# raulmur/ORB_SLAM

Hardware: AMD Instinct MI355X
Metric: frames/s ORB extract+match @640x480, 1000 kp (higher is better)
Workload: dtype u8; 1 GPU; vga: 640x480 grayscale stream, 8 levels, nFeatures 1000, S-blocks frames, extract + Hamming top-2 match vs previous frame (BASELINE.json configs[1] + the frame-to-frame match of the metric); resident_frames_per_gpu=2048, lanes=4, parity_checked_frames=0, parity_mismatches=0, library_build_id=e7130e2d92184036, lane_placement=2

## Files before the change

### orb_slam_amd/csrc/k_select.hip

```cpp
#include <algorithm>
#include <type_traits>

#include "orbx_device.h"
#include "orbx_launch.h"

namespace orbx {

struct QuotaLds { int *nkeys, *nret; uint8_t *thr, *done; };

__global__ __launch_bounds__(64) void k_quota(Batch b) {
    extern __shared__ __attribute__((aligned(16))) uint8_t smem[];
    const DevGeom& g = b.g;
    QuotaLds q;
    q.nkeys = reinterpret_cast<int*>(smem);
    q.nret = q.nkeys + g.quota_cells;
    q.thr = reinterpret_cast<uint8_t*>(q.nret + g.quota_cells);
    q.done = q.thr + g.quota_cells;
    const int frame = blockIdx.x / g.nlevels, level = blockIdx.x - frame * g.nlevels;
    const int lane = (int)threadIdx.x;
    const LevelGeom& L = g.lv[level];
    const CellGeom* cg = b.cells + L.cell_base;
    const CellState* cs = b.cstate + (long long)frame * g.nbands_total;
    CellSel* sel = b.csel + (long long)frame * g.ncells_total + L.cell_base;
    const int nCells = L.ncells, nfc = L.nfeat_cell;
    int dist = 0, nomore = 0;
    for (int c = lane; c < nCells; c += 64) {
        const CellGeom cgc = cg[c];
        int n_hi = 0, n_lo = 0;
        for (int k = 0; k < cgc.nbands; k++) { const CellState t = cs[cgc.band0 + k]; n_hi += t.n_hi; n_lo += t.n_lo; }
        const bool fallback = n_hi <= 3;
        const int nk = cgc.skipped ? 0 : (fallback ? n_lo : n_hi);
        q.thr[c] = (uint8_t)(cgc.skipped || !fallback ? g.fast_th : 7);
        q.nkeys[c] = nk;
        if (cgc.skipped) { q.nret[c] = 0; q.done[c] = 0; }
        else if (nk > nfc) { q.nret[c] = nfc; q.done[c] = 0; }
        else { q.nret[c] = nk; dist += nfc - nk; q.done[c] = 1; nomore++; }
    }
    int nToDistribute = wave_sum(dist), nNoMore = wave_sum(nomore);
    while (nToDistribute > 0 && nNoMore < nCells) {
        const int nNew = nfc + (int)ceilf((float)nToDistribute / (float)(nCells - nNoMore));
        dist = 0; nomore = 0;
        for (int c = lane; c < nCells; c += 64) {
            if (q.done[c]) continue;
            const int nk = q.nkeys[c];
            if (nk > nNew) q.nret[c] = nNew;
            else { q.nret[c] = nk; dist += nNew - nk; q.done[c] = 1; nomore++; }
        }
        nToDistribute = wave_sum(dist);
        nNoMore += wave_sum(nomore);
    }
    int total = 0;
    for (int c0 = 0; c0 < nCells; c0 += 64) total += (c0 + lane < nCells) ? q.nret[c0 + lane] : 0;
    total = wave_sum(total);
    const bool bad = total > L.sel_cap;
    int base = 0;
    for (int c0 = 0; c0 < nCells; c0 += 64) {
        const int c = c0 + lane;
        const int v = c < nCells ? q.nret[c] : 0;
        const int incl = wave_scan_inclusive(v);
        if (c < nCells) {
            CellSel r;
            r.thr = q.thr[c]; r.nkeys = q.nkeys[c];
            r.nretain = bad ? 0 : v;
            r.out_off = bad ? 0 : base + incl - v;
            sel[c] = r;
        }
        base += __builtin_amdgcn_readlane(incl, 63);
    }
    if (lane == 0) {
        if (bad) b.status[frame] = ORBX_ERR_CAPACITY;
        b.level_total[frame * MAX_LEVELS + level] = bad ? 0 : total;
    }
}

struct RespGreater {
    __host__ __device__ constexpr bool operator()(const Cand& x, const Cand& y) const { return x.resp > y.resp; }
};


__device__ __forceinline__ int mask_rank(unsigned long long m) {
// ... 152 lines not shown
            const int Iy = (p[step] - p[-step]) * 2 + (p[step - 1] - p[-step - 1]) + (p[step + 1] - p[-step + 1]);
            a += Ix * Ix;
            bb += Iy * Iy;
            c += Ix * Iy;
        }
    if (fp_contract) {
        const float cc = (float)c * (float)c, sum = (float)a + (float)bb;
        return __builtin_fmaf(-sum, 0.04f * sum, __builtin_fmaf((float)a, (float)bb, -cc)) * scale_sq_sq;
    }
    return ((float)a * (float)bb - (float)c * (float)c - 0.04f * ((float)a + (float)bb) * ((float)a + (float)bb)) * scale_sq_sq;
}

constexpr int SEL_SMALL = 384;
__host__ __device__ constexpr int sel_wave_bytes(int entries) { return (entries * ((int)sizeof(Cand) + 4) + 16 + 15) & ~15; }
template <bool GATHER>
__device__ __forceinline__ bool cell_select_body(const Batch& b, int frame, int cell, int level, uint8_t* smem, int lds_entries, int min_entries, int lane) {
    const DevGeom& g = b.g;
    const LevelGeom& L = g.lv[level];
    const CellGeom cgeo = b.cells[cell];
    const CellSel s = b.csel[(long long)frame * g.ncells_total + cell];
    if (s.nretain <= 0) return true;
    const CellState* bst = b.cstate + (long long)frame * g.nbands_total + cgeo.band0;
    const BandGeom* bgs = b.bands + cgeo.band0;
    Cand* lbase = b.cand + (long long)frame * g.frame_cands + L.cand_base;
    Cand* c = lbase + cgeo.cand_off;
    int n_all = 0;
    for (int k = 0; k < cgeo.nbands; k++) n_all += bst[k].n_all;
    if (n_all < min_entries || (n_all > lds_entries && lds_entries < g.sel_lds_entries)) return false;
    Cand* out = b.sel + (long long)frame * g.frame_sel + L.sel_base + s.out_off;
    const float thr = (float)s.thr;
    long long stride;
    const uint8_t* img = plain_plane<GATHER>(b, L, level, frame, stride);
    if (n_all > lds_entries) {
        if (lane == 0) {
            int m = 0;
            for (int k = 0; k < cgeo.nbands; k++) {
                const Cand* bc = lbase + bgs[k].cand_off;
                const int nb = bst[k].n_all;
                for (int i = 0; i < nb; i++) { const Cand e = bc[i]; if (e.resp >= thr) c[m++] = e; }
            }
            if (g.score_type == ORBX_HARRIS_SCORE)
                for (int i = 0; i < m; i++) c[i].resp = harris_response(img, stride, c[i].pos & 0xFFFF, c[i].pos >> 16, g.fp_contract);
            if (m > s.nretain) std::nth_element(c, c + s.nretain, c + m, RespGreater());
            const int keep = min(m, s.nretain);
            for (int i = 0; i < keep; i++) out[i] = c[i];
        }
        return true;
    }
    Cand* lst = reinterpret_cast<Cand*>(smem);
    uint16_t* lpos = reinterpret_cast<uint16_t*>(smem + (size_t)lds_entries * sizeof(Cand));
    uint16_t* rpos = lpos + lds_entries;
    const unsigned long long lt = (1ull << lane) - 1ull;
    int m = 0;
    for (int k = 0; k < cgeo.nbands; k++) {
        const Cand* bc = lbase + bgs[k].cand_off;
        const int nb = bst[k].n_all;
        for (int base = 0; base < nb; base += 256) {
            Cand e4[4];
#pragma unroll
            for (int k = 0; k < 4; k++) {
                const int i = base + 64 * k + lane;
                e4[k].pos = 0; e4[k].resp = -1.f;
                if (i < nb) e4[k] = bc[i];
            }
#pragma unroll
            for (int k = 0; k < 4; k++) {
                if (base + 64 * k >= nb) break;
                const int i = base + 64 * k + lane;
                const bool pass = i < nb && e4[k].resp >= thr;
                const unsigned long long mk = __ballot(pass);
                if (pass) lst[m + __popcll(mk & lt)] = e4[k];
                m += __popcll(mk);
            }
        }
    }
    wave_lds_fence();
    if (g.score_type == ORBX_HARRIS_SCORE) {
        for (int i = lane; i < m; i += 64) lst[i].resp = harris_response(img, stride, lst[i].pos & 0xFFFF, lst[i].pos >> 16, g.fp_contract);
        wave_lds_fence();
    }
    if (m > s.nretain) wave_nth_element(lst, 0, s.nretain, m, lpos, rpos, lane);
    const int keep = min(m, s.nretain);
    for (int i = lane; i < keep; i += 64) out[i] = lst[i];
    return true;
}

template <bool GATHER>
__device__ __forceinline__ void k_cell_select_body(const Batch& b, int lds_entries) {
    extern __shared__ __attribute__((aligned(16))) uint8_t smem[];
    const DevGeom& g = b.g;
    const int wave = wave_id(), lane = (int)threadIdx.x & 63;
    const int id = (int)blockIdx.x * 4 + wave;
    if (id >= b.nframes * g.ncells_total) return;
    const int frame = id / g.ncells_total, cell = id - frame * g.ncells_total;
    const bool done = cell_select_body<GATHER>(b, frame, cell, find_level(g.cell_bases, cell), smem + wave * sel_wave_bytes(lds_entries), lds_entries, 0, lane);
    if (lane == 0) b.long_cells[id] = done ? 0 : 1;
}
__global__ __launch_bounds__(256) void k_cell_select(Batch b, int lds_entries) { k_cell_select_body<false>(b, lds_entries); }
__global__ __launch_bounds__(256) void k_cell_select_gather(Batch b, int lds_entries) { k_cell_select_body<true>(b, lds_entries); }
#ifndef ORBX_SEL_LONG_CHUNK
#define ORBX_SEL_LONG_CHUNK 8
#endif
constexpr int SEL_LONG_CHUNK = ORBX_SEL_LONG_CHUNK, SEL_LONG_WAVES = 4;
__host__ __device__ constexpr int sel_long_bytes(int entries) {
    int m = 0;
    for (int share = 1; share <= 4; share++) { const int v = share * sel_wave_bytes((entries + share - 1) / share); m = v > m ? v : m; }
    return m;
}
template <bool GATHER>
__device__ __forceinline__ void k_cell_select_long_body(const Batch& b) {
    extern __shared__ __attribute__((aligned(16))) uint8_t smem[];
    const DevGeom& g = b.g;
    const int lane = (int)threadIdx.x & 63, wave = wave_id(), total = b.nframes * g.ncells_total;
    const int id0 = (int)blockIdx.x * SEL_LONG_CHUNK;
    static_assert(SEL_LONG_CHUNK <= 64, "one flag per lane");
    const int quarter = (g.sel_lds_entries + 3) / 4, third = (g.sel_lds_entries + 2) / 3, half = (g.sel_lds_entries + 1) / 2;
    int n_all = 0;
    const bool mine = lane < SEL_LONG_CHUNK && id0 + lane < total && b.long_cells[id0 + lane] != 0;
    if (mine) {
        const int id = id0 + lane, frame = id / g.ncells_total, cell = id - frame * g.ncells_total;
        const CellGeom cgeo = b.cells[cell];
        const CellState* bst = b.cstate + (long long)frame * g.nbands_total + cgeo.band0;
        for (int k = 0; k < cgeo.nbands; k++) n_all += bst[k].n_all;
    }
    const unsigned long long mQ = __ballot(mine && n_all <= quarter), mT = __ballot(mine && n_all > quarter && n_all <= third),
                             mH = __ballot(mine && n_all > third && n_all <= half), mF = __ballot(mine && n_all > half);
    if (!(mQ | mT | mH | mF)) return;
    const unsigned long long cls_m[4] = {mQ, mT, mH, mF};
    const int cls_share[4] = {4, 3, 2, 1}, cls_entries[4] = {quarter, third, half, g.sel_lds_entries};
#pragma unroll 1
    for (int c = 0; c < 4; c++) {
        unsigned long long m = cls_m[c];
        const int share = cls_share[c], entries = cls_entries[c];
        if (!m) continue;
        if (wave < share) {
            uint8_t* area = smem + wave * sel_wave_bytes(entries);
            for (int r = 0; m; r++) {
                const int id = id0 + __ffsll((long long)m) - 1;
                m &= m - 1;
                if (r % share != wave) continue;
                const int frame = id / g.ncells_total, cell = id - frame * g.ncells_total;
                (void)cell_select_body<GATHER>(b, frame, cell, find_level(g.cell_bases, cell), area, entries, 0, lane);
                wave_lds_fence();
            }
        }
        __syncthreads();
    }
}
__global__ __launch_bounds__(SEL_LONG_WAVES * 64) void k_cell_select_long(Batch b) { k_cell_select_long_body<false>(b); }
__global__ __launch_bounds__(SEL_LONG_WAVES * 64) void k_cell_select_long_gather(Batch b) { k_cell_select_long_body<true>(b); }

__device__ __forceinline__ void level_select_body(const Batch& b, int frame, int level, uint8_t* smem, int lane) {
    const DevGeom& g = b.g;
    const LevelGeom& L = g.lv[level];
    const int total = b.level_total[frame * MAX_LEVELS + level];
    int n = total;
    if (total > L.ndesired) {
        n = L.ndesired;
        if (n > 0) {
            Cand* v = b.sel + (long long)frame * g.frame_sel + L.sel_base;
            if (total > g.sel_lds_entries) {
                if (lane == 0) std::nth_element(v, v + n, v + total, RespGreater());
            } else {
                Cand* lst = reinterpret_cast<Cand*>(smem);
                uint16_t* lpos = reinterpret_cast<uint16_t*>(smem + (size_t)g.sel_lds_entries * sizeof(Cand));
                uint16_t* rpos = lpos + g.sel_lds_entries;
                for (int i0 = 0; i0 < total; i0 += 256) {
                    Cand e[4];
#pragma unroll
                    for (int k = 0; k < 4; k++) { const int i = i0 + 64 * k + lane; if (i < total) e[k] = v[i]; }
#pragma unroll
                    for (int k = 0; k < 4; k++) { const int i = i0 + 64 * k + lane; if (i < total) lst[i] = e[k]; }
                }
                wave_lds_fence();
                wave_nth_element(lst, 0, n, total, lpos, rpos, lane);
                for (int i = lane; i < n; i += 64) v[i] = lst[i];
            }
        }
    }
    if (lane == 0) b.level_count[frame * MAX_LEVELS + level] = n;
}

__global__ __launch_bounds__(64) void k_level_select(Batch b) {
    extern __shared__ __attribute__((aligned(16))) uint8_t smem[];
    const DevGeom& g = b.g;
    const int frame = blockIdx.x / g.nlevels, level = blockIdx.x - frame * g.nlevels;
    level_select_body(b, frame, level, smem, (int)threadIdx.x);
}

__global__ __launch_bounds__(64) void k_debug_nth(const float* resp, int n, int nth, int* out_idx) {
    extern __shared__ __attribute__((aligned(16))) uint8_t smem[];
    Cand* lst = reinterpret_cast<Cand*>(smem);
    uint16_t* lpos = reinterpret_cast<uint16_t*>(smem + (size_t)n * sizeof(Cand));
    uint16_t* rpos = lpos + n;
    const int lane = threadIdx.x;
    for (int i = lane; i < n; i += 64) { Cand e; e.pos = (uint32_t)i; e.resp = resp[i]; lst[i] = e; }
    wave_lds_fence();
    wave_nth_element(lst, 0, nth, n, lpos, rpos, lane);
    for (int i = lane; i < n; i += 64) out_idx[i] = (int)lst[i].pos;
}
int launch_debug_nth(const float* d_resp, int n, int nth, int* d_out) {
    const size_t lds = (size_t)n * (sizeof(Cand) + 4) + 16;
    if (lds > 160 * 1024) return ORBX_ERR_ARG;
    if (lds > 64 * 1024 && hipFuncSetAttribute(reinterpret_cast<const void*>(&k_debug_nth), hipFuncAttributeMaxDynamicSharedMemorySize, (int)lds) != hipSuccess) return ORBX_ERR_DEVICE;
    hipLaunchKernelGGL(k_debug_nth, dim3(1), dim3(64), lds, 0, d_resp, n, nth, d_out);
    return hipGetLastError() == hipSuccess ? ORBX_OK : ORBX_ERR_DEVICE;
}


int launch_quota(const Batch& b, const HostGeom& hg, hipStream_t stream) {
    const DevGeom& g = hg.g;
    const size_t lds = (size_t)g.quota_cells * QUOTA_LDS_PER_CELL;
    if (lds > 64 * 1024 && hipFuncSetAttribute(reinterpret_cast<const void*>(&k_quota), hipFuncAttributeMaxDynamicSharedMemorySize, (int)lds) != hipSuccess) return ORBX_ERR_DEVICE;
    hipLaunchKernelGGL(k_quota, dim3(b.nframes * g.nlevels), dim3(64), lds, stream, b);
    ORBX_LAUNCH_CHECK();
    return ORBX_OK;
}

int launch_cell_select(const Batch& b, const HostGeom& hg, hipStream_t stream) {
    const DevGeom& g = hg.g;
    const int F = b.nframes;
    const int small = F < PYR_FUSED_MAX_FRAMES ? g.sel_lds_entries : std::min(SEL_SMALL, g.sel_lds_entries);
    const size_t lds = (size_t)4 * sel_wave_bytes(small);
    auto* const ksel = b.img_tab ? k_cell_select_gather : k_cell_select;
    if (lds > 64 * 1024 && hipFuncSetAttribute(reinterpret_cast<const void*>(ksel), hipFuncAttributeMaxDynamicSharedMemorySize, (int)lds) != hipSuccess) return ORBX_ERR_DEVICE;
    hipLaunchKernelGGL(ksel, dim3((F * g.ncells_total + 3) / 4), dim3(256), lds, stream, b, small);
    ORBX_LAUNCH_CHECK();
    if (small < g.sel_lds_entries) {
        const size_t ldsl = (size_t)sel_long_bytes(g.sel_lds_entries);
        auto* const klong = b.img_tab ? k_cell_select_long_gather : k_cell_select_long;
        if (ldsl > 64 * 1024 && hipFuncSetAttribute(reinterpret_cast<const void*>(klong), hipFuncAttributeMaxDynamicSharedMemorySize, (int)ldsl) != hipSuccess) return ORBX_ERR_DEVICE;
        hipLaunchKernelGGL(klong, dim3((F * g.ncells_total + SEL_LONG_CHUNK - 1) / SEL_LONG_CHUNK), dim3(SEL_LONG_WAVES * 64), ldsl, stream, b);
        ORBX_LAUNCH_CHECK();
    }
    return ORBX_OK;
}

int launch_level_select(const Batch& b, const HostGeom& hg, hipStream_t stream) {
    const DevGeom& g = hg.g;
    const size_t lds = (size_t)g.sel_lds_level;
    if (lds > 64 * 1024 && hipFuncSetAttribute(reinterpret_cast<const void*>(&k_level_select), hipFuncAttributeMaxDynamicSharedMemorySize, (int)lds) != hipSuccess) return ORBX_ERR_DEVICE;
    hipLaunchKernelGGL(k_level_select, dim3(b.nframes * g.nlevels), dim3(64), lds, stream, b);
    ORBX_LAUNCH_CHECK();
    return ORBX_OK;
}

}
```

### orb_slam_amd/csrc/orbx_api.hip

```cpp
#include <climits>
#include <cstdio>
#include <cstdlib>
#include <cstring>

#include "orbx_internal.h"

namespace orbx {
int launch_eval_math(int kind, const float* in0, const float* in1, float* out0, float* out1, int n);
int launch_eval_compass(const uint32_t* c, const uint32_t* e, const uint32_t* w, const uint32_t* nn, const uint32_t* ss, uint32_t* out, int n, int t);
int launch_eval_blur_window(const uint8_t* win, uint8_t* out, int n, int ties_even, int general);
void stage_timer_collect(StageTimer& t);
int launch_debug_nth(const float* d_resp, int n, int nth, int* d_out);
int launch_ingest(uint8_t* d_dst, const uint8_t* mapped_src, size_t bytes, hipStream_t stream);
}
using namespace orbx;

struct orbx_extractor {
    orbx_params p;
    std::string err;
    int gw = 0, gh = 0;
    HostGeom hg;
    struct __attribute__((visibility("hidden"))) Geom {
        DevBuf cells, bands, tabx, taby, pyr_tab;
        DevBuf pyr, blur, cand, sel, cstate, csel, level_total, level_count, status, long_cells;
    } geo;
    bool fallback_hint = true;
    DevBuf d_img1;
    PinnedBuf h_img1;
    DevBuf d_out1;
    PinnedBuf h_out1;
    bool zero_copy = true;
    Stream s1;
    int stop_after = -1;
    bool no_xcd_affinity = false;
    int od_min_frames = ORBX_OD_MIN_FRAMES_DEFAULT;
    int blur_on_demand = ORBX_BLUR_ON_DEMAND_DEFAULT;
    StageTimer timer;
    SideStream side;
    Batch last;
// ... 37 lines not shown

static int ensure_geometry(orbx_extractor* h, int w, int hgt) {
    if (h->gw == w && h->gh == hgt) return ORBX_OK;
    HIPCHK(h, hipDeviceSynchronize());
    h->geo = {};
    h->gw = h->gh = 0;
    h->have_last = false;
    HostGeom hg;
    int rc = build_geometry(h->p, w, hgt, hg, h->err);
    if (rc != ORBX_OK) return rc;
    h->hg = hg;
    const DevGeom& g = h->hg.g;
    const size_t B = (size_t)h->p.max_batch;
    orbx_extractor::Geom& d = h->geo;
    if ((rc = upload(h, d.cells, h->hg.cells)) != ORBX_OK) return rc;
    if ((rc = upload(h, d.bands, h->hg.bands)) != ORBX_OK) return rc;
    if ((rc = upload(h, d.tabx, h->hg.tabx)) != ORBX_OK) return rc;
    if ((rc = upload(h, d.taby, h->hg.taby)) != ORBX_OK) return rc;
    if ((rc = upload(h, d.pyr_tab, h->hg.pyr_tab)) != ORBX_OK) return rc;
    HIPCHK(h, d.pyr.ensure(B * g.frame_plane_bytes));
    HIPCHK(h, d.blur.ensure(B * g.frame_plane_bytes));
    HIPCHK(h, d.cand.ensure(B * std::max(g.frame_cands, 1) * sizeof(Cand)));
    HIPCHK(h, d.sel.ensure((B * std::max(g.frame_sel, 1) + 4) * sizeof(Cand)));
    HIPCHK(h, d.cstate.ensure(B * g.nbands_total * sizeof(CellState)));
    HIPCHK(h, hipMemset(d.cstate, 0, B * g.nbands_total * sizeof(CellState)));
    HIPCHK(h, d.csel.ensure(B * g.ncells_total * sizeof(CellSel)));
    HIPCHK(h, d.level_total.ensure(B * MAX_LEVELS * sizeof(int32_t)));
    HIPCHK(h, d.level_count.ensure(B * MAX_LEVELS * sizeof(int32_t)));
    HIPCHK(h, hipMemset(d.level_total, 0, B * MAX_LEVELS * sizeof(int32_t)));
    HIPCHK(h, hipMemset(d.level_count, 0, B * MAX_LEVELS * sizeof(int32_t)));
    HIPCHK(h, d.status.ensure(B * sizeof(int32_t)));
    HIPCHK(h, d.long_cells.ensure((B * g.ncells_total + 64) * sizeof(int32_t)));
    HIPCHK(h, hipDeviceSynchronize());
    h->gw = w;
    h->gh = hgt;
    return ORBX_OK;
}

static void fill_batch(orbx_extractor* h, Batch& b) {
    const orbx_extractor::Geom& d = h->geo;
    b.g = h->hg.g; b.cells = d.cells.as<CellGeom>(); b.bands = d.bands.as<BandGeom>(); b.tabx = d.tabx.as<ResizeX>(); b.taby = d.taby.as<ResizeY>();
    b.pyr_tab = d.pyr_tab.as<int>(); b.pyr = d.pyr.as(); b.blur = d.blur.as();
    b.cand = d.cand.as<Cand>(); b.sel = d.sel.as<Cand>(); b.cstate = d.cstate.as<CellState>(); b.csel = d.csel.as<CellSel>();
    b.level_total = d.level_total.as<int32_t>(); b.level_count = d.level_count.as<int32_t>(); b.status = d.status.as<int32_t>();
    b.long_cells = d.long_cells.as<int32_t>();
}

static void group_batch(orbx_extractor* h, Batch& b, int f0, int n, orbx_keypoint* d_kps, uint8_t* d_desc, int32_t* d_n, int cap, int32_t* d_status) {
    memset(&b, 0, sizeof(b));
    fill_batch(h, b);
    b.fallback_hint = h->fallback_hint ? 1 : 0;
    b.nframes = n;
    b.xcd_affinity = (b.nframes >= XCD_AFFINITY_MIN_FRAMES && !h->no_xcd_affinity) ? 1 : 0;
    b.blur_on_demand = h->blur_on_demand;
    b.od_min_frames = h->od_min_frames;
    b.out_kps = d_kps + (size_t)f0 * cap;
    b.out_desc = d_desc + (size_t)f0 * cap * 32;
    b.out_n = d_n + f0;
// ... 813 lines not shown
```

### orb_slam_amd/csrc/orbx_device.h

```cpp
#pragma once
#include <hip/hip_runtime.h>

#include "orb_math.h"
#include "orbx_internal.h"

namespace orbx {

static __device__ __constant__ uint32_t c_pattern[256] = {
#include "orb_pattern_packed.inc"
};

__device__ __forceinline__ const uint8_t* level0_src(const Batch& b, int frame, long long& stride) {
    typedef const ImgSrc __attribute__((address_space(4)))* ctab_t;
    const ctab_t e = (ctab_t)(uintptr_t)b.img_tab + frame;
    stride = e->row_stride;
    return e->data;
}

template <bool GATHER = false>
__device__ __forceinline__ const uint8_t* plain_plane(const Batch& b, const LevelGeom& L, int level, int frame, long long& stride) {
    if (level == 0) {
        if constexpr (GATHER) return level0_src(b, frame, stride);
        stride = b.img_row_stride;
        return b.img + (long long)frame * b.img_frame_stride;
// ... 22 lines not shown
        item = block - frame * per_frame;
    }
    return frame < b.nframes;
}
__device__ __forceinline__ bool frame_item_magic(const Batch& b, unsigned block, unsigned per_frame, unsigned magic, int& frame, int& item) {
    const unsigned slot = b.xcd_affinity ? block >> 3 : block;
    unsigned fr = magic ? __umulhi(slot, magic) : slot;
    if (fr * per_frame > slot) --fr;
    frame = (int)(b.xcd_affinity ? fr * 8u + (block & 7u) : fr);
    item = (int)(slot - fr * per_frame);
    return frame < b.nframes;
}
static inline int frame_item_blocks(const Batch& b, int per_frame) {
    return (b.xcd_affinity ? (b.nframes + 7) / 8 * 8 : b.nframes) * per_frame;
}

constexpr unsigned long long UMAX_NIBBLES = 0x3689ABCDDEEEFFFFull;

__device__ __forceinline__ int wave_scan_inclusive(int v) {
    v += __builtin_amdgcn_update_dpp(0, v, 0x111, 0xf, 0xf, false);
    v += __builtin_amdgcn_update_dpp(0, v, 0x112, 0xf, 0xf, false);
    v += __builtin_amdgcn_update_dpp(0, v, 0x114, 0xf, 0xf, false);
    v += __builtin_amdgcn_update_dpp(0, v, 0x118, 0xf, 0xf, false);
    v += __builtin_amdgcn_update_dpp(0, v, 0x142, 0xa, 0xf, false);
    v += __builtin_amdgcn_update_dpp(0, v, 0x143, 0xc, 0xf, false);
    return v;
}

__device__ __forceinline__ int wave_sum(int v) { return __builtin_amdgcn_readlane(wave_scan_inclusive(v), 63); }

// ... 33 lines not shown
```

### orb_slam_amd/csrc/orbx_geometry.hip

```cpp
#include <cfloat>
#include <climits>
#include <cmath>
#include <cstdlib>
#include <cstring>

#include "orbx_internal.h"

namespace orbx {

static inline int round_even(double v) { return (int)std::lrint(v); }
static inline int floor_int(double v) { int i = (int)v; return i - (i > v); }
static inline int ceil_int(double v) { int i = (int)v; return i + (i < v); }
static inline int16_t sat16(float v) {
    int iv = round_even(v);
    return (int16_t)(iv < SHRT_MIN ? SHRT_MIN : iv > SHRT_MAX ? SHRT_MAX : iv);
}
static inline int align_up(int v, int a) { return (v + a - 1) / a * a; }

static int build_geometry_band(const orbx_params& p, int w, int h, HostGeom& out, std::string& err, const int band_px, const FastShape& shape) {
    const int threads = shape.threads;
    const int nl = p.nlevels;
    if (nl < 1 || nl > MAX_LEVELS) { err = "nlevels out of range [1,16]"; return ORBX_ERR_ARG; }
    if (p.nfeatures < 1) { err = "nfeatures must be >= 1"; return ORBX_ERR_ARG; }
    if (!(p.scale_factor > 1.0f) || p.scale_factor > 2.5f) { err = "scale_factor must be in (1, 2.5]"; return ORBX_ERR_ARG; }
// ... 134 lines not shown
                    bg.cand_off = cand_off;
                    bg.cand_cap = ((cw + 1) / 2) * ((bh + 1) / 2);
                    if (cw > 0) {
                        const int nd = fast_row_dwords((bg.x0 - 3) & 3, cw);
                        bg.inv_nd = 1.0f / (float)nd;
                        bg.inv_s = 1.0f / (float)(nd * 4);
                        bg.inv_cpr = 1.0f / (float)(nd >> 2);
                    }
                    cand_off += bg.cand_cap;
                    c.cand_cap += bg.cand_cap;
                    c.nbands++;
                    out.bands.push_back(bg);
                }
                out.cells.push_back(c);
            }
        cell_base += L.ncells;
        cand_base += cand_off;
        L.sel_base = sel_base;
        L.sel_cap = std::min(cand_off, L.ncells * L.nfeat_cell + L.ncells * L.ncells + L.ndesired + 64);
        sel_base += L.sel_cap;
        L.slot_base = slot_base;
        slot_base += L.ndesired;
        L.quad_base = quad_base;
        quad_base += (L.ndesired + 3) / 4;

        L.btiles_x = (L.w + 247) / 248;
        L.btiles_y = (L.h + BLUR_ROWS - 1) / BLUR_ROWS;
        L.btile_base = btile_base;
        btile_base += L.btiles_x * L.btiles_y;
        L.btiles_y_s = (L.h + BLUR_ROWS_SMALL - 1) / BLUR_ROWS_SMALL;
// ... 214 lines not shown
```

### orb_slam_amd/csrc/orbx_internal.h

```cpp
#pragma once
#include <hip/hip_runtime.h>
#include <stdint.h>
#include <string>
#include <vector>

#include "orbx.h"
#include "orbx_host.h"

namespace orbx {

constexpr int MAX_LEVELS = 16;
constexpr int EDGE = 16;
constexpr int HALF_PATCH = 15;

struct Cand {
    uint32_t pos;
    float resp;
};

struct ResizeX { int16_t sx, sx1, a0, a1; };
struct ResizeY { int16_t sy0, sy1, b0, b1; };

struct LevelGeom {
    int w, h;
// ... 106 lines not shown
struct PyrGroup {
    int l0, depth;
    int ntx, nty;
    int xtab, ytab;
    int lds_off[PYR_MAX_DEPTH];
    int pitch[PYR_MAX_DEPTH];
    int lds_bytes;
};
#ifndef ORBX_PYR_TILE
#define ORBX_PYR_TILE 16, 16
#endif

constexpr int QUOTA_LDS_PER_CELL = 10;
constexpr int QUOTA_MAX_CELLS = 160 * 1024 / QUOTA_LDS_PER_CELL / 64 * 64;
struct CellState { int32_t n_all, n_hi, n_lo, thr; };
struct CellSel { int32_t thr, nkeys, nretain, out_off; };

struct DevGeom {
    int nlevels;
    int ncells_total;
    int nbands_total;
    uint32_t nbands_magic;
    int nbtiles_total, nbtiles_total_s;
    int nmb_total;
    int nslots;
    int nquads;
    int quota_cells;
    int score_type, fast_th, tmin;
    int fp_contract;
    int frame_plane_bytes;
    int frame_cands;
// ... 6 lines not shown
    PyrGroup pyr[PYR_MAX_GROUPS];
    int umax[HALF_PATCH + 1];
    int cell_bases[MAX_LEVELS], quad_bases[MAX_LEVELS], btile_bases[MAX_LEVELS], btile_bases_s[MAX_LEVELS], mb_bases[MAX_LEVELS];
    LevelGeom lv[MAX_LEVELS];
};

struct ImgSrc {
    const uint8_t* data;
    long long row_stride;
};
static_assert(sizeof(ImgSrc) == 16, "one scalar dwordx4 per table entry");

struct Batch {
    DevGeom g;
    const CellGeom* cells;
    const BandGeom* bands;
    const ResizeX* tabx;
    const ResizeY* taby;
    const int* pyr_tab;
    const uint8_t* img;
    long long img_row_stride, img_frame_stride;
    uint8_t* pyr;
    uint8_t* blur;
    Cand* cand;
    Cand* sel;
    CellState* cstate;
    int fallback_hint;
    CellSel* csel;
    int32_t* level_total;
    int32_t* level_count;
    int32_t* status;
    int32_t* long_cells;
    orbx_keypoint* out_kps;
    uint8_t* out_desc;
    int32_t* out_n;
    int32_t* out_status;
    int cap;
    int nframes;
    int xcd_affinity;
    int od_min_frames;
    int blur_on_demand;
    const ImgSrc* img_tab;
    unsigned long long img_tab_bits;
// ... 18 lines not shown
    int cpr, items;
};
static inline int pix_channels(int fmt) {
    switch (fmt) {
        case ORBX_PIX_GRAY8: return 1;
        case ORBX_PIX_RGB8: case ORBX_PIX_BGR8: return 3;
        case ORBX_PIX_RGBA8: case ORBX_PIX_BGRA8: return 4;
        default: return 0;
    }
}
int launch_to_gray(const ColorArgs& a, int nframes, int fmt, hipStream_t stream);

struct HostGeom {
    DevGeom g;
    std::vector<CellGeom> cells;
    std::vector<BandGeom> bands;
    std::vector<ResizeX> tabx;
    std::vector<ResizeY> taby;
    std::vector<int> pyr_tab;
    std::vector<int> features_per_level;
    std::vector<float> scale, inv_scale;
};

int build_geometry(const orbx_params& p, int w, int h, HostGeom& out, std::string& err);

enum Stage { ST_PYRAMID = 0, ST_FAST_CELLS, ST_QUOTA, ST_CELL_SELECT, ST_LEVEL_SELECT, ST_BLUR, ST_DESCRIBE, ST_COUNT };

struct StageTimer {
    bool enabled = false;
    std::vector<hipEvent_t> pool;
// ... 16 lines not shown
```

Measured before the change: 473,700 frames/s.

## Precompute per-cell records and pass band counts from quota to cell select

```diff
diff --git a/orb_slam_amd/csrc/k_select.hip b/orb_slam_amd/csrc/k_select.hip
--- a/orb_slam_amd/csrc/k_select.hip
+++ b/orb_slam_amd/csrc/k_select.hip
@@ -8,31 +8,47 @@
 
 struct QuotaLds { int *nkeys, *nret; uint8_t *thr, *done; };
 
-__global__ __launch_bounds__(64) void k_quota(Batch b) {
+__global__ __launch_bounds__(64) void k_quota(Batch b, unsigned magic) {
     extern __shared__ __attribute__((aligned(16))) uint8_t smem[];
     const DevGeom& g = b.g;
+    asm volatile("" ::"s"(b.xcd_affinity), "s"(b.nframes), "s"(g.nlevels), "s"(g.quota_cells), "s"(b.cellrec), "s"(b.cstate), "s"(b.csel), "s"(b.cbands),
+                 "s"(g.ncells_total), "s"(g.nbands_total), "s"(g.fast_th));
+    int frame, level;
+    if (!frame_item_magic(b, blockIdx.x, (unsigned)g.nlevels, magic, frame, level)) return;
     QuotaLds q;
     q.nkeys = reinterpret_cast<int*>(smem);
     q.nret = q.nkeys + g.quota_cells;
     q.thr = reinterpret_cast<uint8_t*>(q.nret + g.quota_cells);
     q.done = q.thr + g.quota_cells;
-    const int frame = blockIdx.x / g.nlevels, level = blockIdx.x - frame * g.nlevels;
     const int lane = (int)threadIdx.x;
     const LevelGeom& L = g.lv[level];
-    const CellGeom* cg = b.cells + L.cell_base;
+    const CellRec* rec = b.cellrec + L.cell_base;
     const CellState* cs = b.cstate + (long long)frame * g.nbands_total;
     CellSel* sel = b.csel + (long long)frame * g.ncells_total + L.cell_base;
+    CellBands* sbn = b.cbands + (long long)frame * g.ncells_total + L.cell_base;
     const int nCells = L.ncells, nfc = L.nfeat_cell;
     int dist = 0, nomore = 0;
     for (int c = lane; c < nCells; c += 64) {
-        const CellGeom cgc = cg[c];
-        int n_hi = 0, n_lo = 0;
-        for (int k = 0; k < cgc.nbands; k++) { const CellState t = cs[cgc.band0 + k]; n_hi += t.n_hi; n_lo += t.n_lo; }
+        const int nb = rec[c].nbands, skipped = rec[c].skipped, band0 = rec[c].band0;
+        CellState t[CELL_REC_BANDS];
+#pragma unroll
+        for (int k = 0; k < CELL_REC_BANDS; k++) { t[k].n_all = 0; t[k].n_hi = 0; t[k].n_lo = 0; t[k].thr = 0; if (k < nb) t[k] = cs[band0 + k]; }
+        int n_hi = 0, n_lo = 0, n_all = 0;
+#pragma unroll
+        for (int k = 0; k < CELL_REC_BANDS; k++) { n_hi += t[k].n_hi; n_lo += t[k].n_lo; n_all += t[k].n_all; }
+        if (nb > 1) {
+            CellBands bn;
+#pragma unroll
+            for (int k = 0; k < CELL_REC_BANDS; k++) bn.n[k] = t[k].n_all;
+            sbn[c] = bn;
+        }
+        for (int k = CELL_REC_BANDS; k < nb; k++) { const CellState u = cs[band0 + k]; n_hi += u.n_hi; n_lo += u.n_lo; n_all += u.n_all; }
+        sel[c].n_all = n_all;
         const bool fallback = n_hi <= 3;
-        const int nk = cgc.skipped ? 0 : (fallback ? n_lo : n_hi);
-        q.thr[c] = (uint8_t)(cgc.skipped || !fallback ? g.fast_th : 7);
+        const int nk = skipped ? 0 : (fallback ? n_lo : n_hi);
+        q.thr[c] = (uint8_t)(skipped || !fallback ? g.fast_th : 7);
         q.nkeys[c] = nk;
-        if (cgc.skipped) { q.nret[c] = 0; q.done[c] = 0; }
+        if (skipped) { q.nret[c] = 0; q.done[c] = 0; }
         else if (nk > nfc) { q.nret[c] = nfc; q.done[c] = 0; }
         else { q.nret[c] = nk; dist += nfc - nk; q.done[c] = 1; nomore++; }
     }
@@ -59,11 +75,9 @@
         const int v = c < nCells ? q.nret[c] : 0;
         const int incl = wave_scan_inclusive(v);
         if (c < nCells) {
-            CellSel r;
-            r.thr = q.thr[c]; r.nkeys = q.nkeys[c];
-            r.nretain = bad ? 0 : v;
-            r.out_off = bad ? 0 : base + incl - v;
-            sel[c] = r;
+            sel[c].thr = q.thr[c];
+            sel[c].nretain = bad ? 0 : v;
+            sel[c].out_off = bad ? 0 : base + incl - v;
         }
         base += __builtin_amdgcn_readlane(incl, 63);
     }
@@ -246,29 +260,40 @@
 constexpr int SEL_SMALL = 384;
 __host__ __device__ constexpr int sel_wave_bytes(int entries) { return (entries * ((int)sizeof(Cand) + 4) + 16 + 15) & ~15; }
 template <bool GATHER>
-__device__ __forceinline__ bool cell_select_body(const Batch& b, int frame, int cell, int level, uint8_t* smem, int lds_entries, int min_entries, int lane) {
-    const DevGeom& g = b.g;
-    const LevelGeom& L = g.lv[level];
-    const CellGeom cgeo = b.cells[cell];
-    const CellSel s = b.csel[(long long)frame * g.ncells_total + cell];
+__device__ __forceinline__ const uint8_t* cell_plane(const Batch& b, const CellRec& rc, int frame, long long& stride) {
+    if (rc.level == 0) {
+        if constexpr (GATHER) return level0_src(b, frame, stride);
+        stride = b.img_row_stride;
+        return b.img + (long long)frame * b.img_frame_stride;
+    }
+    stride = rc.stride;
+    return b.pyr + (long long)frame * b.g.frame_plane_bytes + rc.plane_off;
+}
+template <bool GATHER>
+__device__ __forceinline__ bool cell_select_body(const Batch& b, int frame, int cell, uint8_t* smem, int lds_entries, int lane) {
+    const DevGeom& g = b.g;
+    CellRec rc;
+    CellSel s;
+    CellBands bn;
+    load_cell_records(b, cell, (long long)frame * g.ncells_total + cell, rc, s, bn);
     if (s.nretain <= 0) return true;
-    const CellState* bst = b.cstate + (long long)frame * g.nbands_total + cgeo.band0;
-    const BandGeom* bgs = b.bands + cgeo.band0;
-    Cand* lbase = b.cand + (long long)frame * g.frame_cands + L.cand_base;
-    Cand* c = lbase + cgeo.cand_off;
-    int n_all = 0;
-    for (int k = 0; k < cgeo.nbands; k++) n_all += bst[k].n_all;
-    if (n_all < min_entries || (n_all > lds_entries && lds_entries < g.sel_lds_entries)) return false;
-    Cand* out = b.sel + (long long)frame * g.frame_sel + L.sel_base + s.out_off;
+    const int n_all = s.n_all;
+    if (n_all > lds_entries && lds_entries < g.sel_lds_entries) return false;
+    Cand* fcand = b.cand + (long long)frame * g.frame_cands;
+    Cand* out = b.sel + (long long)frame * g.frame_sel + rc.sel_base + s.out_off;
     const float thr = (float)s.thr;
-    long long stride;
-    const uint8_t* img = plain_plane<GATHER>(b, L, level, frame, stride);
+    const bool listed = rc.nbands <= CELL_REC_BANDS;
+    auto band_list = [&](int k) { return fcand + g.lv[rc.level].cand_base + b.bands[rc.band0 + k].cand_off; };
+    auto band_len = [&](int k) { return b.cstate[(long long)frame * g.nbands_total + rc.band0 + k].n_all; };
     if (n_all > lds_entries) {
         if (lane == 0) {
+            long long stride;
+            const uint8_t* img = cell_plane<GATHER>(b, rc, frame, stride);
+            Cand* c = fcand + rc.cand_off;
             int m = 0;
-            for (int k = 0; k < cgeo.nbands; k++) {
-                const Cand* bc = lbase + bgs[k].cand_off;
-                const int nb = bst[k].n_all;
+            for (int k = 0; k < rc.nbands; k++) {
+                const Cand* bc = band_list(k);
+                const int nb = band_len(k);
                 for (int i = 0; i < nb; i++) { const Cand e = bc[i]; if (e.resp >= thr) c[m++] = e; }
             }
             if (g.score_type == ORBX_HARRIS_SCORE)
@@ -284,9 +309,7 @@
     uint16_t* rpos = lpos + lds_entries;
     const unsigned long long lt = (1ull << lane) - 1ull;
     int m = 0;
-    for (int k = 0; k < cgeo.nbands; k++) {
-        const Cand* bc = lbase + bgs[k].cand_off;
-        const int nb = bst[k].n_all;
+    auto take_band = [&](const Cand* bc, int nb) {
         for (int base = 0; base < nb; base += 256) {
             Cand e4[4];
 #pragma unroll
@@ -305,9 +328,20 @@
                 m += __popcll(mk);
             }
         }
+    };
+    if (listed) {
+#pragma unroll
+        for (int k = 0; k < CELL_REC_BANDS; k++) {
+            if (k >= rc.nbands) break;
+            take_band(fcand + rc.band_cand[k], rc.nbands == 1 ? s.n_all : bn.n[k]);
+        }
+    } else {
+        for (int k = 0; k < rc.nbands; k++) take_band(band_list(k), band_len(k));
     }
     wave_lds_fence();
     if (g.score_type == ORBX_HARRIS_SCORE) {
+        long long stride;
+        const uint8_t* img = cell_plane<GATHER>(b, rc, frame, stride);
         for (int i = lane; i < m; i += 64) lst[i].resp = harris_response(img, stride, lst[i].pos & 0xFFFF, lst[i].pos >> 16, g.fp_contract);
         wave_lds_fence();
     }
@@ -318,18 +352,21 @@
 }
 
 template <bool GATHER>
-__device__ __forceinline__ void k_cell_select_body(const Batch& b, int lds_entries) {
+__device__ __forceinline__ void k_cell_select_body(const Batch& b, int lds_entries, unsigned magic) {
     extern __shared__ __attribute__((aligned(16))) uint8_t smem[];
     const DevGeom& g = b.g;
     const int wave = wave_id(), lane = (int)threadIdx.x & 63;
-    const int id = (int)blockIdx.x * 4 + wave;
-    if (id >= b.nframes * g.ncells_total) return;
-    const int frame = id / g.ncells_total, cell = id - frame * g.ncells_total;
-    const bool done = cell_select_body<GATHER>(b, frame, cell, find_level(g.cell_bases, cell), smem + wave * sel_wave_bytes(lds_entries), lds_entries, 0, lane);
-    if (lane == 0) b.long_cells[id] = done ? 0 : 1;
-}
-__global__ __launch_bounds__(256) void k_cell_select(Batch b, int lds_entries) { k_cell_select_body<false>(b, lds_entries); }
-__global__ __launch_bounds__(256) void k_cell_select_gather(Batch b, int lds_entries) { k_cell_select_body<true>(b, lds_entries); }
+    asm volatile("" ::"s"(b.xcd_affinity), "s"(b.nframes), "s"(g.ncells_total), "s"(b.cellrec), "s"(b.csel), "s"(b.cbands), "s"(g.sel_lds_entries), "s"(b.cand),
+                 "s"(b.sel), "s"(g.frame_cands), "s"(g.frame_sel), "s"(b.long_cells));
+    int frame, item;
+    if (!frame_item_magic(b, blockIdx.x, (unsigned)(g.ncells_total + 3) >> 2, magic, frame, item)) return;
+    const int cell = item * 4 + wave;
+    if (cell >= g.ncells_total) return;
+    const bool done = cell_select_body<GATHER>(b, frame, cell, smem + wave * sel_wave_bytes(lds_entries), lds_entries, lane);
+    if (lane == 0) b.long_cells[frame * g.ncells_total + cell] = done ? 0 : 1;
+}
+__global__ __launch_bounds__(256) __attribute__((amdgpu_waves_per_eu(8, 8))) void k_cell_select(Batch b, int lds_entries, unsigned magic) { k_cell_select_body<false>(b, lds_entries, magic); }
+__global__ __launch_bounds__(256) __attribute__((amdgpu_waves_per_eu(8, 8))) void k_cell_select_gather(Batch b, int lds_entries, unsigned magic) { k_cell_select_body<true>(b, lds_entries, magic); }
 #ifndef ORBX_SEL_LONG_CHUNK
 #define ORBX_SEL_LONG_CHUNK 8
 #endif
@@ -339,27 +376,14 @@
     for (int share = 1; share <= 4; share++) { const int v = share * sel_wave_bytes((entries + share - 1) / share); m = v > m ? v : m; }
     return m;
 }
-template <bool GATHER>
-__device__ __forceinline__ void k_cell_select_long_body(const Batch& b) {
-    extern __shared__ __attribute__((aligned(16))) uint8_t smem[];
-    const DevGeom& g = b.g;
-    const int lane = (int)threadIdx.x & 63, wave = wave_id(), total = b.nframes * g.ncells_total;
-    const int id0 = (int)blockIdx.x * SEL_LONG_CHUNK;
-    static_assert(SEL_LONG_CHUNK <= 64, "one flag per lane");
-    const int quarter = (g.sel_lds_entries + 3) / 4, third = (g.sel_lds_entries + 2) / 3, half = (g.sel_lds_entries + 1) / 2;
-    int n_all = 0;
-    const bool mine = lane < SEL_LONG_CHUNK && id0 + lane < total && b.long_cells[id0 + lane] != 0;
-    if (mine) {
-        const int id = id0 + lane, frame = id / g.ncells_total, cell = id - frame * g.ncells_total;
-        const CellGeom cgeo = b.cells[cell];
-        const CellState* bst = b.cstate + (long long)frame * g.nbands_total + cgeo.band0;
-        for (int k = 0; k < cgeo.nbands; k++) n_all += bst[k].n_all;
-    }
-    const unsigned long long mQ = __ballot(mine && n_all <= quarter), mT = __ballot(mine && n_all > quarter && n_all <= third),
-                             mH = __ballot(mine && n_all > third && n_all <= half), mF = __ballot(mine && n_all > half);
+template <class Take>
+__device__ __forceinline__ void shared_area_select(bool mine, int n, int sel_lds_entries, uint8_t* smem, int wave, Take take) {
+    const int quarter = (sel_lds_entries + 3) / 4, third = (sel_lds_entries + 2) / 3, half = (sel_lds_entries + 1) / 2;
+    const unsigned long long mQ = __ballot(mine && n <= quarter), mT = __ballot(mine && n > quarter && n <= third),
+                             mH = __ballot(mine && n > third && n <= half), mF = __ballot(mine && n > half);
     if (!(mQ | mT | mH | mF)) return;
     const unsigned long long cls_m[4] = {mQ, mT, mH, mF};
-    const int cls_share[4] = {4, 3, 2, 1}, cls_entries[4] = {quarter, third, half, g.sel_lds_entries};
+    const int cls_share[4] = {4, 3, 2, 1}, cls_entries[4] = {quarter, third, half, sel_lds_entries};
 #pragma unroll 1
     for (int c = 0; c < 4; c++) {
         unsigned long long m = cls_m[c];
@@ -368,56 +392,83 @@
         if (wave < share) {
             uint8_t* area = smem + wave * sel_wave_bytes(entries);
             for (int r = 0; m; r++) {
-                const int id = id0 + __ffsll((long long)m) - 1;
+                const int item = __ffsll((long long)m) - 1;
                 m &= m - 1;
                 if (r % share != wave) continue;
-                const int frame = id / g.ncells_total, cell = id - frame * g.ncells_total;
-                (void)cell_select_body<GATHER>(b, frame, cell, find_level(g.cell_bases, cell), area, entries, 0, lane);
+                take(item, area, entries);
                 wave_lds_fence();
             }
         }
         __syncthreads();
     }
 }
-__global__ __launch_bounds__(SEL_LONG_WAVES * 64) void k_cell_select_long(Batch b) { k_cell_select_long_body<false>(b); }
-__global__ __launch_bounds__(SEL_LONG_WAVES * 64) void k_cell_select_long_gather(Batch b) { k_cell_select_long_body<true>(b); }
-
-__device__ __forceinline__ void level_select_body(const Batch& b, int frame, int level, uint8_t* smem, int lane) {
-    const DevGeom& g = b.g;
-    const LevelGeom& L = g.lv[level];
-    const int total = b.level_total[frame * MAX_LEVELS + level];
-    int n = total;
-    if (total > L.ndesired) {
-        n = L.ndesired;
-        if (n > 0) {
-            Cand* v = b.sel + (long long)frame * g.frame_sel + L.sel_base;
-            if (total > g.sel_lds_entries) {
-                if (lane == 0) std::nth_element(v, v + n, v + total, RespGreater());
-            } else {
-                Cand* lst = reinterpret_cast<Cand*>(smem);
-                uint16_t* lpos = reinterpret_cast<uint16_t*>(smem + (size_t)g.sel_lds_entries * sizeof(Cand));
-                uint16_t* rpos = lpos + g.sel_lds_entries;
-                for (int i0 = 0; i0 < total; i0 += 256) {
-                    Cand e[4];
-#pragma unroll
-                    for (int k = 0; k < 4; k++) { const int i = i0 + 64 * k + lane; if (i < total) e[k] = v[i]; }
-#pragma unroll
-                    for (int k = 0; k < 4; k++) { const int i = i0 + 64 * k + lane; if (i < total) lst[i] = e[k]; }
-                }
-                wave_lds_fence();
-                wave_nth_element(lst, 0, n, total, lpos, rpos, lane);
-                for (int i = lane; i < n; i += 64) v[i] = lst[i];
-            }
-        }
-    }
-    if (lane == 0) b.level_count[frame * MAX_LEVELS + level] = n;
-}
-
-__global__ __launch_bounds__(64) void k_level_select(Batch b) {
+template <bool GATHER>
+__device__ __forceinline__ void k_cell_select_long_body(const Batch& b, unsigned magic) {
     extern __shared__ __attribute__((aligned(16))) uint8_t smem[];
     const DevGeom& g = b.g;
-    const int frame = blockIdx.x / g.nlevels, level = blockIdx.x - frame * g.nlevels;
-    level_select_body(b, frame, level, smem, (int)threadIdx.x);
+    const int lane = (int)threadIdx.x & 63, wave = wave_id();
+    static_assert(SEL_LONG_CHUNK <= 64, "one flag per lane");
+    asm volatile("" ::"s"(b.xcd_affinity), "s"(b.nframes), "s"(g.ncells_total), "s"(b.long_cells), "s"(g.sel_lds_entries));
+    int frame, item;
+    if (!frame_item_magic(b, blockIdx.x, (unsigned)(g.ncells_total + SEL_LONG_CHUNK - 1) / SEL_LONG_CHUNK, magic, frame, item)) return;
+    const int cell0 = item * SEL_LONG_CHUNK;
+    const long long id = (long long)frame * g.ncells_total + cell0 + lane;
+    const bool mine = lane < SEL_LONG_CHUNK && cell0 + lane < g.ncells_total && b.long_cells[id] != 0;
+    const int n_all = mine ? b.csel[id].n_all : 0;
+    shared_area_select(mine, n_all, g.sel_lds_entries, smem, wave, [&](int i, uint8_t* area, int entries) {
+        (void)cell_select_body<GATHER>(b, frame, cell0 + i, area, entries, lane);
+    });
+}
+__global__ __launch_bounds__(SEL_LONG_WAVES * 64) void k_cell_select_long(Batch b, unsigned magic) { k_cell_select_long_body<false>(b, magic); }
+__global__ __launch_bounds__(SEL_LONG_WAVES * 64) void k_cell_select_long_gather(Batch b, unsigned magic) { k_cell_select_long_body<true>(b, magic); }
+
+__device__ __forceinline__ void level_select_body(const Batch& b, int frame, int level, int total, int n, uint8_t* smem, int entries, int lane) {
+    const DevGeom& g = b.g;
+    Cand* v = b.sel + (long long)frame * g.frame_sel + g.lv[level].sel_base;
+    if (total > entries) {
+        if (lane == 0) std::nth_element(v, v + n, v + total, RespGreater());
+        return;
+    }
+    Cand* lst = reinterpret_cast<Cand*>(smem);
+    uint16_t* lpos = reinterpret_cast<uint16_t*>(smem + (size_t)entries * sizeof(Cand));
+    uint16_t* rpos = lpos + entries;
+    for (int i0 = 0; i0 < total; i0 += 256) {
+        Cand e[4];
+#pragma unroll
+        for (int k = 0; k < 4; k++) { const int i = i0 + 64 * k + lane; if (i < total) e[k] = v[i]; }
+#pragma unroll
+        for (int k = 0; k < 4; k++) { const int i = i0 + 64 * k + lane; if (i < total) lst[i] = e[k]; }
+    }
+    wave_lds_fence();
+    wave_nth_element(lst, 0, n, total, lpos, rpos, lane);
+    for (int i = lane; i < n; i += 64) v[i] = lst[i];
+}
+
+constexpr int LSEL_CHUNK = 4, LSEL_WAVES = 4;
+__global__ __launch_bounds__(LSEL_WAVES * 64) void k_level_select(Batch b, unsigned magic) {
+    extern __shared__ __attribute__((aligned(16))) uint8_t smem[];
+    const DevGeom& g = b.g;
+    const int lane = (int)threadIdx.x & 63, wave = wave_id();
+    asm volatile("" ::"s"(b.xcd_affinity), "s"(b.nframes), "s"(g.nlevels), "s"(b.level_total), "s"(b.level_count), "s"(g.sel_lds_entries), "s"(b.sel),
+                 "s"(g.frame_sel));
+    int frame, item;
+    if (!frame_item_magic(b, blockIdx.x, (unsigned)(g.nlevels + LSEL_CHUNK - 1) / LSEL_CHUNK, magic, frame, item)) return;
+    const int level0 = item * LSEL_CHUNK;
+    const bool valid = lane < LSEL_CHUNK && level0 + lane < g.nlevels;
+    int total = 0, nd = 0;
+    if (valid) { total = b.level_total[frame * MAX_LEVELS + level0 + lane]; nd = g.lv[level0 + lane].ndesired; }
+    if (valid && wave == 0) b.level_count[frame * MAX_LEVELS + level0 + lane] = total > nd ? nd : total;
+    shared_area_select(valid && total > nd && nd > 0, total, g.sel_lds_entries, smem, wave, [&](int i, uint8_t* area, int entries) {
+        level_select_body(b, frame, level0 + i, __builtin_amdgcn_readlane(total, i), __builtin_amdgcn_readlane(nd, i), area, entries, lane);
+    });
+}
+__global__ __launch_bounds__(64) void k_level_select_one(Batch b) {
+    extern __shared__ __attribute__((aligned(16))) uint8_t smem[];
+    const DevGeom& g = b.g;
+    const int frame = blockIdx.x / g.nlevels, level = blockIdx.x - frame * g.nlevels, lane = (int)threadIdx.x;
+    const int total = b.level_total[frame * MAX_LEVELS + level], nd = g.lv[level].ndesired;
+    if (lane == 0) b.level_count[frame * MAX_LEVELS + level] = total > nd ? nd : total;
+    if (total > nd && nd > 0) level_select_body(b, frame, level, total, nd, smem, g.sel_lds_entries, lane);
 }
 
 __global__ __launch_bounds__(64) void k_debug_nth(const float* resp, int n, int nth, int* out_idx) {
@@ -444,7 +495,7 @@
     const DevGeom& g = hg.g;
     const size_t lds = (size_t)g.quota_cells * QUOTA_LDS_PER_CELL;
     if (lds > 64 * 1024 && hipFuncSetAttribute(reinterpret_cast<const void*>(&k_quota), hipFuncAttributeMaxDynamicSharedMemorySize, (int)lds) != hipSuccess) return ORBX_ERR_DEVICE;
-    hipLaunchKernelGGL(k_quota, dim3(b.nframes * g.nlevels), dim3(64), lds, stream, b);
+    hipLaunchKernelGGL(k_quota, dim3(frame_item_blocks(b, g.nlevels)), dim3(64), lds, stream, b, frame_item_magic_of(g.nlevels));
     ORBX_LAUNCH_CHECK();
     return ORBX_OK;
 }
@@ -456,13 +507,15 @@
     const size_t lds = (size_t)4 * sel_wave_bytes(small);
     auto* const ksel = b.img_tab ? k_cell_select_gather : k_cell_select;
     if (lds > 64 * 1024 && hipFuncSetAttribute(reinterpret_cast<const void*>(ksel), hipFuncAttributeMaxDynamicSharedMemorySize, (int)lds) != hipSuccess) return ORBX_ERR_DEVICE;
-    hipLaunchKernelGGL(ksel, dim3((F * g.ncells_total + 3) / 4), dim3(256), lds, stream, b, small);
+    const int per4 = (g.ncells_total + 3) / 4;
+    hipLaunchKernelGGL(ksel, dim3(frame_item_blocks(b, per4)), dim3(256), lds, stream, b, small, frame_item_magic_of(per4));
     ORBX_LAUNCH_CHECK();
     if (small < g.sel_lds_entries) {
         const size_t ldsl = (size_t)sel_long_bytes(g.sel_lds_entries);
         auto* const klong = b.img_tab ? k_cell_select_long_gather : k_cell_select_long;
         if (ldsl > 64 * 1024 && hipFuncSetAttribute(reinterpret_cast<const void*>(klong), hipFuncAttributeMaxDynamicSharedMemorySize, (int)ldsl) != hipSuccess) return ORBX_ERR_DEVICE;
-        hipLaunchKernelGGL(klong, dim3((F * g.ncells_total + SEL_LONG_CHUNK - 1) / SEL_LONG_CHUNK), dim3(SEL_LONG_WAVES * 64), ldsl, stream, b);
+        const int perl = (g.ncells_total + SEL_LONG_CHUNK - 1) / SEL_LONG_CHUNK;
+        hipLaunchKernelGGL(klong, dim3(frame_item_blocks(b, perl)), dim3(SEL_LONG_WAVES * 64), ldsl, stream, b, frame_item_magic_of(perl));
         ORBX_LAUNCH_CHECK();
     }
     return ORBX_OK;
@@ -470,9 +523,16 @@
 
 int launch_level_select(const Batch& b, const HostGeom& hg, hipStream_t stream) {
     const DevGeom& g = hg.g;
-    const size_t lds = (size_t)g.sel_lds_level;
-    if (lds > 64 * 1024 && hipFuncSetAttribute(reinterpret_cast<const void*>(&k_level_select), hipFuncAttributeMaxDynamicSharedMemorySize, (int)lds) != hipSuccess) return ORBX_ERR_DEVICE;
-    hipLaunchKernelGGL(k_level_select, dim3(b.nframes * g.nlevels), dim3(64), lds, stream, b);
+    if (b.nframes < PYR_FUSED_MAX_FRAMES) {
+        const size_t lds = (size_t)g.sel_lds_level;
+        if (lds > 64 * 1024 && hipFuncSetAttribute(reinterpret_cast<const void*>(&k_level_select_one), hipFuncAttributeMaxDynamicSharedMemorySize, (int)lds) != hipSuccess) return ORBX_ERR_DEVICE;
+        hipLaunchKernelGGL(k_level_select_one, dim3(b.nframes * g.nlevels), dim3(64), lds, stream, b);
+    } else {
+        const size_t lds = (size_t)sel_long_bytes(g.sel_lds_entries);
+        if (lds > 64 * 1024 && hipFuncSetAttribute(reinterpret_cast<const void*>(&k_level_select), hipFuncAttributeMaxDynamicSharedMemorySize, (int)lds) != hipSuccess) return ORBX_ERR_DEVICE;
+        const int per = (g.nlevels + LSEL_CHUNK - 1) / LSEL_CHUNK;
+        hipLaunchKernelGGL(k_level_select, dim3(frame_item_blocks(b, per)), dim3(LSEL_WAVES * 64), lds, stream, b, frame_item_magic_of(per));
+    }
     ORBX_LAUNCH_CHECK();
     return ORBX_OK;
 }
diff --git a/orb_slam_amd/csrc/orbx_api.hip b/orb_slam_amd/csrc/orbx_api.hip
--- a/orb_slam_amd/csrc/orbx_api.hip
+++ b/orb_slam_amd/csrc/orbx_api.hip
@@ -21,8 +21,8 @@
     int gw = 0, gh = 0;
     HostGeom hg;
     struct __attribute__((visibility("hidden"))) Geom {
-        DevBuf cells, bands, tabx, taby, pyr_tab;
-        DevBuf pyr, blur, cand, sel, cstate, csel, level_total, level_count, status, long_cells;
+        DevBuf cells, cellrecs, bands, tabx, taby, pyr_tab;
+        DevBuf pyr, blur, cand, sel, cstate, csel, cbands, level_total, level_count, status, long_cells;
     } geo;
     bool fallback_hint = true;
     DevBuf d_img1;
@@ -90,6 +90,7 @@
     const size_t B = (size_t)h->p.max_batch;
     orbx_extractor::Geom& d = h->geo;
     if ((rc = upload(h, d.cells, h->hg.cells)) != ORBX_OK) return rc;
+    if ((rc = upload(h, d.cellrecs, h->hg.cellrecs)) != ORBX_OK) return rc;
     if ((rc = upload(h, d.bands, h->hg.bands)) != ORBX_OK) return rc;
     if ((rc = upload(h, d.tabx, h->hg.tabx)) != ORBX_OK) return rc;
     if ((rc = upload(h, d.taby, h->hg.taby)) != ORBX_OK) return rc;
@@ -101,6 +102,8 @@
     HIPCHK(h, d.cstate.ensure(B * g.nbands_total * sizeof(CellState)));
     HIPCHK(h, hipMemset(d.cstate, 0, B * g.nbands_total * sizeof(CellState)));
     HIPCHK(h, d.csel.ensure(B * g.ncells_total * sizeof(CellSel)));
+    HIPCHK(h, d.cbands.ensure(B * g.ncells_total * sizeof(CellBands)));
+    HIPCHK(h, hipMemset(d.cbands, 0, B * g.ncells_total * sizeof(CellBands)));
     HIPCHK(h, d.level_total.ensure(B * MAX_LEVELS * sizeof(int32_t)));
     HIPCHK(h, d.level_count.ensure(B * MAX_LEVELS * sizeof(int32_t)));
     HIPCHK(h, hipMemset(d.level_total, 0, B * MAX_LEVELS * sizeof(int32_t)));
@@ -115,9 +118,9 @@
 
 static void fill_batch(orbx_extractor* h, Batch& b) {
     const orbx_extractor::Geom& d = h->geo;
-    b.g = h->hg.g; b.cells = d.cells.as<CellGeom>(); b.bands = d.bands.as<BandGeom>(); b.tabx = d.tabx.as<ResizeX>(); b.taby = d.taby.as<ResizeY>();
+    b.g = h->hg.g; b.cells = d.cells.as<CellGeom>(); b.cellrec = d.cellrecs.as<CellRec>(); b.bands = d.bands.as<BandGeom>(); b.tabx = d.tabx.as<ResizeX>(); b.taby = d.taby.as<ResizeY>();
     b.pyr_tab = d.pyr_tab.as<int>(); b.pyr = d.pyr.as(); b.blur = d.blur.as();
-    b.cand = d.cand.as<Cand>(); b.sel = d.sel.as<Cand>(); b.cstate = d.cstate.as<CellState>(); b.csel = d.csel.as<CellSel>();
+    b.cand = d.cand.as<Cand>(); b.sel = d.sel.as<Cand>(); b.cstate = d.cstate.as<CellState>(); b.csel = d.csel.as<CellSel>(); b.cbands = d.cbands.as<CellBands>();
     b.level_total = d.level_total.as<int32_t>(); b.level_count = d.level_count.as<int32_t>(); b.status = d.status.as<int32_t>();
     b.long_cells = d.long_cells.as<int32_t>();
 }
diff --git a/orb_slam_amd/csrc/orbx_device.h b/orb_slam_amd/csrc/orbx_device.h
--- a/orb_slam_amd/csrc/orbx_device.h
+++ b/orb_slam_amd/csrc/orbx_device.h
@@ -60,6 +60,25 @@
 static inline int frame_item_blocks(const Batch& b, int per_frame) {
     return (b.xcd_affinity ? (b.nframes + 7) / 8 * 8 : b.nframes) * per_frame;
 }
+static inline unsigned frame_item_magic_of(int per_frame) {
+    return per_frame > 1 ? (unsigned)((1ull << 32) / (unsigned)per_frame) + 1u : 0u;
+}
+
+typedef int rec16_t __attribute__((ext_vector_type(16)));
+typedef int rec8_t __attribute__((ext_vector_type(8)));
+typedef int rec4_t __attribute__((ext_vector_type(4)));
+__device__ __forceinline__ void load_cell_records(const Batch& b, int cell, long long frame_cell, CellRec& rc, CellSel& s, CellBands& bn) {
+    typedef const rec16_t __attribute__((address_space(4)))* c16_t;
+    typedef const rec8_t __attribute__((address_space(4)))* c8_t;
+    typedef const rec4_t __attribute__((address_space(4)))* c4_t;
+    rec16_t vr = *((c16_t)(uintptr_t)b.cellrec + cell);
+    rec4_t vs = *((c4_t)(uintptr_t)b.csel + frame_cell);
+    rec8_t vb = *((c8_t)(uintptr_t)b.cbands + frame_cell);
+    asm volatile("" : "+s"(vr), "+s"(vs), "+s"(vb));
+    rc = __builtin_bit_cast(CellRec, vr);
+    s = __builtin_bit_cast(CellSel, vs);
+    bn = __builtin_bit_cast(CellBands, vb);
+}
 
 constexpr unsigned long long UMAX_NIBBLES = 0x3689ABCDDEEEFFFFull;
 
diff --git a/orb_slam_amd/csrc/orbx_geometry.hip b/orb_slam_amd/csrc/orbx_geometry.hip
--- a/orb_slam_amd/csrc/orbx_geometry.hip
+++ b/orb_slam_amd/csrc/orbx_geometry.hip
@@ -172,6 +172,16 @@
                 }
                 out.cells.push_back(c);
             }
+        for (int ci = L.cell_base; ci < L.cell_base + L.ncells; ci++) {
+            const CellGeom& c = out.cells[ci];
+            CellRec r;
+            memset(&r, 0, sizeof(r));
+            r.level = l; r.nbands = c.nbands; r.skipped = c.skipped; r.band0 = c.band0;
+            r.sel_base = sel_base; r.plane_off = L.plane_off; r.stride = L.stride;
+            r.cand_off = L.cand_base + c.cand_off;
+            for (int k = 0; k < c.nbands && k < CELL_REC_BANDS; k++) r.band_cand[k] = L.cand_base + out.bands[c.band0 + k].cand_off;
+            out.cellrecs.push_back(r);
+        }
         cell_base += L.ncells;
         cand_base += cand_off;
         L.sel_base = sel_base;
diff --git a/orb_slam_amd/csrc/orbx_internal.h b/orb_slam_amd/csrc/orbx_internal.h
--- a/orb_slam_amd/csrc/orbx_internal.h
+++ b/orb_slam_amd/csrc/orbx_internal.h
@@ -144,7 +144,17 @@
 constexpr int QUOTA_LDS_PER_CELL = 10;
 constexpr int QUOTA_MAX_CELLS = 160 * 1024 / QUOTA_LDS_PER_CELL / 64 * 64;
 struct CellState { int32_t n_all, n_hi, n_lo, thr; };
-struct CellSel { int32_t thr, nkeys, nretain, out_off; };
+constexpr int CELL_REC_BANDS = 8;
+struct alignas(64) CellRec {
+    int32_t level, nbands, skipped, band0;
+    int32_t sel_base;
+    int32_t plane_off, stride;
+    int32_t cand_off;
+    int32_t band_cand[CELL_REC_BANDS];
+};
+struct alignas(16) CellSel { int32_t n_all, thr, nretain, out_off; };
+struct alignas(32) CellBands { int32_t n[CELL_REC_BANDS]; };
+static_assert(sizeof(CellRec) == 64 && sizeof(CellSel) == 16 && sizeof(CellBands) == 32, "one scalar load per record");
 
 struct DevGeom {
     int nlevels;
@@ -181,6 +191,7 @@
 struct Batch {
     DevGeom g;
     const CellGeom* cells;
+    const CellRec* cellrec;
     const BandGeom* bands;
     const ResizeX* tabx;
     const ResizeY* taby;
@@ -194,6 +205,7 @@
     CellState* cstate;
     int fallback_hint;
     CellSel* csel;
+    CellBands* cbands;
     int32_t* level_total;
     int32_t* level_count;
     int32_t* status;
@@ -242,6 +254,7 @@
 struct HostGeom {
     DevGeom g;
     std::vector<CellGeom> cells;
+    std::vector<CellRec> cellrecs;
     std::vector<BandGeom> bands;
     std::vector<ResizeX> tabx;
     std::vector<ResizeY> taby;
```

New measurement: 480,900 frames/s (median of 6 runs). +1.5%, better.
